# alibaba/EasyParallelLibrary

Hardware: AMD Instinct MI355X
Metric: samples_per_sec (higher is better)
Workload: dtype bf16; 1 GPU; model=bert-large, global_batch=128, seq_len=512, parallelism=dp1

## Files before the change

### csrc/kernels/attention.hip

```cpp

#include <hip/hip_runtime.h>
#include <cstdint>
#include <cstdlib>
#include <cstring>
#include <type_traits>

#include "attn_lds_image.h"

using bf16x8 = __attribute__((ext_vector_type(8))) short;
using bf16x4 = __attribute__((ext_vector_type(4))) short;
using f32x16 = __attribute__((ext_vector_type(16))) float;
using i32x2 = __attribute__((ext_vector_type(2))) int;
using u32x2 = __attribute__((ext_vector_type(2))) unsigned int;
using f32x2 = __attribute__((ext_vector_type(2))) float;
using f32x4 = __attribute__((ext_vector_type(4))) float;
using bf16v2 = __attribute__((ext_vector_type(2))) __bf16;

#define DEVI __device__ __forceinline__

namespace {

DEVI float bf2f(short u) {
  union { unsigned int i; float f; } v;
  v.i = ((unsigned int)(unsigned short)u) << 16;
  return v.f;
}

DEVI unsigned short f2bf(float f) {
  union { float f; unsigned int i; } v;
  v.f = f;
  unsigned int lsb = (v.i >> 16) & 1u;
  return (unsigned short)((v.i + 0x7fffu + lsb) >> 16);
}

DEVI unsigned int pack2(float a, float b) {
  return (unsigned int)f2bf(a) | ((unsigned int)f2bf(b) << 16);
}

DEVI int crow(int r, int hi) {
  return (r & 3) + 8 * (r >> 2) + 4 * hi;
}

DEVI unsigned int cvt_pk_bf16(float a, float b) {
  f32x2 f = {a, b};
  return __builtin_bit_cast(unsigned int,
                            __builtin_convertvector(f, bf16v2));
}

template <bool HW = false>
DEVI bf16x8 assemble_pfrag(const float* p) {
  unsigned int c0 = HW ? cvt_pk_bf16(p[0], p[1]) : pack2(p[0], p[1]);
  unsigned int c1 = HW ? cvt_pk_bf16(p[2], p[3]) : pack2(p[2], p[3]);
  unsigned int c2 = HW ? cvt_pk_bf16(p[4], p[5]) : pack2(p[4], p[5]);
  unsigned int c3 = HW ? cvt_pk_bf16(p[6], p[7]) : pack2(p[6], p[7]);
  i32x2 r = __builtin_amdgcn_permlane32_swap((int)c0, (int)c2, false, false);
  i32x2 s = __builtin_amdgcn_permlane32_swap((int)c1, (int)c3, false, false);
  union { unsigned int d[4]; bf16x8 v; } out;
  out.d[0] = (unsigned int)r[0];
  out.d[1] = (unsigned int)s[0];
  out.d[2] = (unsigned int)r[1];
  out.d[3] = (unsigned int)s[1];
  return out.v;
}

using attn_img::img_off;
using attn_img::img_pitch;
using attn_img::tr_frag;

template <bool TR, int D>
DEVI short* img_at(short (&img)[64][TR ? img_pitch<D>() : D + 8], int row,
                   int col) {
  return TR ? &img[0][0] + img_off<D>(row, col >> 3) : &img[row][col];
}

DEVI f32x16 load_rowconst(const float* c32, int hi) {
  f32x16 out;
#pragma unroll
  for (int g = 0; g < 4; ++g) {
    const f32x4 v = *reinterpret_cast<const f32x4*>(c32 + 8 * g + 4 * hi);
    out[4 * g + 0] = v[0];
    out[4 * g + 1] = v[1];
    out[4 * g + 2] = v[2];
    out[4 * g + 3] = v[3];
  }
  return out;
}

struct RowMask {
  int lo, hi_;
  DEVI RowMask(int64_t q0, int64_t seq, int64_t mykv, int causal) {
    const int64_t rows = seq - q0;
    hi_ = mykv >= seq ? 0 : (rows < 32 ? (int)rows : 32);
    const int64_t d = mykv - q0;
    lo = (causal && d > 0) ? (d < 32 ? (int)d : 32) : 0;
  }
  DEVI bool masked(int c) const { return c < lo || c >= hi_; }
};

DEVI void store_acc_bf16(short* p, const f32x16& acc, int hi) {
#pragma unroll
  for (int g = 0; g < 4; ++g) {
    u32x2 v = {cvt_pk_bf16(acc[4 * g], acc[4 * g + 1]),
               cvt_pk_bf16(acc[4 * g + 2], acc[4 * g + 3])};
    *reinterpret_cast<u32x2*>(p + 8 * g + 4 * hi) = v;
  }
}

DEVI int64_t sample_len(const int* seqlens, int64_t b, int64_t seq) {
  if (seqlens == nullptr) return seq;
  const int64_t n = __builtin_amdgcn_readfirstlane(seqlens[b]);
  return n < 0 ? 0 : (n > seq ? seq : n);
}

template <int D>
DEVI void zero_row(short* p, int hi) {
  const u32x2 z = {0u, 0u};
#pragma unroll
  for (int j = 0; j < D / 32; ++j)
#pragma unroll
    for (int g = 0; g < 4; ++g)
      *reinterpret_cast<u32x2*>(p + j * 32 + 8 * g + 4 * hi) = z;
}

DEVI void philox_round(unsigned int& c0, unsigned int& c1,
                       unsigned int& c2, unsigned int& c3,
                       unsigned int k0, unsigned int k1) {
  const unsigned int hi0 = __umulhi(0xD2511F53u, c0);
  const unsigned int lo0 = 0xD2511F53u * c0;
  const unsigned int hi1 = __umulhi(0xCD9E8D57u, c2);
  const unsigned int lo1 = 0xCD9E8D57u * c2;
  c0 = hi1 ^ c1 ^ k0;
  c1 = lo1;
  c2 = hi0 ^ c3 ^ k1;
  c3 = lo0;
}

DEVI void philox4x32(unsigned int c0, unsigned int c1, unsigned int c2,
                     unsigned int c3, unsigned int k0, unsigned int k1,
                     unsigned int out[4]) {
#pragma unroll
  for (int i = 0; i < 10; ++i) {
    philox_round(c0, c1, c2, c3, k0, k1);
    k0 += 0x9E3779B9u;
    k1 += 0xBB67AE85u;
  }
  out[0] = c0; out[1] = c1; out[2] = c2; out[3] = c3;
}


template <bool MASKED, bool DROP, int D>
DEVI void fwd_tile(const short (&ldsK)[64][D + 8],
                   const short (&ldsV)[D][72],
                   int sub, int64_t kvs, int64_t seq, int64_t myq,
                   float scale, int causal, const bf16x8 (&qfrag)[D / 16],
                   f32x16 (&ot)[D / 32], float& m, float& l, int lq,
                   int hi, unsigned int* maskrow, int64_t mask_w,
                   unsigned int seed0, unsigned int seed1,
                   unsigned int bh32, int drop_thresh, float inv_keep) {
  f32x16 st = {};
#pragma unroll
  for (int c = 0; c < D / 16; ++c) {
    bf16x8 kfrag =
        *reinterpret_cast<const bf16x8*>(&ldsK[sub + lq][hi * 8 + 16 * c]);
    st = __builtin_amdgcn_mfma_f32_32x32x16_bf16(kfrag, qfrag[c], st, 0, 0,
                                                 0);
  }
  float s[16];
  float tile_max = -1e30f;
#pragma unroll
  for (int r = 0; r < 16; ++r) {
    float sv = st[r] * scale;
    if (MASKED) {
      const int64_t kvg = kvs + crow(r, hi);
      if (kvg >= seq || (causal && kvg > myq)) sv = -1e30f;
    }
    s[r] = sv;
    tile_max = fmaxf(tile_max, sv);
  }
  tile_max = fmaxf(tile_max, __shfl_xor(tile_max, 32, 64));
  const float m_new = fmaxf(m, tile_max);
  const float alpha = __expf(m - m_new);
  float rowsum = 0.f;
#pragma unroll
  for (int r = 0; r < 16; ++r) {
    s[r] = __expf(s[r] - m_new);
    rowsum += s[r];
  }
  rowsum += __shfl_xor(rowsum, 32, 64);
  l = l * alpha + rowsum;
  m = m_new;
  if (DROP) {
    unsigned int rnd[4];
    philox4x32((unsigned int)myq,
               (unsigned int)(kvs >> 5) * 2u + (unsigned int)hi,
               bh32, 0x2E1B2137u, seed0, seed1, rnd);
    unsigned int mybits = 0;
#pragma unroll
    for (int r = 0; r < 16; ++r) {
      const unsigned int byte = (rnd[r >> 2] >> ((r & 3) * 8)) & 0xFFu;
      const bool keep = (int)byte >= drop_thresh;
      s[r] = keep ? s[r] * inv_keep : 0.f;
      mybits |= (unsigned int)keep << crow(r, hi);
    }
    const unsigned int word = mybits | __shfl_xor(mybits, 32, 64);
    if (hi == 0 && myq < seq)
      maskrow[myq * mask_w + (kvs >> 5)] = word;
  }
#pragma unroll
  for (int j = 0; j < D / 32; ++j)
#pragma unroll
    for (int r = 0; r < 16; ++r)
      ot[j][r] *= alpha;
  bf16x8 pf0 = assemble_pfrag<true>(&s[0]);
  bf16x8 pf1 = assemble_pfrag<true>(&s[8]);
#pragma unroll
  for (int kc = 0; kc < 2; ++kc) {
    bf16x8 pf = kc == 0 ? pf0 : pf1;
#pragma unroll
    for (int j = 0; j < D / 32; ++j) {
      bf16x8 vt = *reinterpret_cast<const bf16x8*>(
          &ldsV[j * 32 + lq][sub + kc * 16 + hi * 8]);
      ot[j] = __builtin_amdgcn_mfma_f32_32x32x16_bf16(vt, pf, ot[j], 0, 0,
                                                      0);
    }
  }
}

template <bool DROP, int D>
__global__ __launch_bounds__(256, D == 64 ? 3 : 2) void attn_fwd_kernel(
    const short* __restrict__ q, const short* __restrict__ k,
    const short* __restrict__ v, short* __restrict__ out,
    float* __restrict__ lse, int64_t seq, float scale, int causal,
    int64_t heads, int64_t in_sb, int64_t in_sh, int64_t in_ss,
    int64_t o_sb, int64_t o_sh, int64_t o_ss,
    unsigned int* __restrict__ mask, int64_t mask_w,
    unsigned long long seed, int drop_thresh, float inv_keep,
    const int* __restrict__ seqlens) {
  __shared__ short ldsV[2][D][72];
  __shared__ short ldsK[2][64][D + 8];
  const int lane = threadIdx.x & 63;
  const int wave = threadIdx.x >> 6;
  const int hi = lane >> 5;
  const int lq = lane & 31;
  const int64_t bh = causal ? (int64_t)blockIdx.x : (int64_t)blockIdx.y;
  const int64_t boff = (bh / heads) * in_sb + (bh % heads) * in_sh;
  const int64_t qb = causal ? (int64_t)gridDim.y - 1 - blockIdx.y
                            : (int64_t)blockIdx.x;
  const int64_t q0_blk = qb * 128;
  const int64_t q0 = q0_blk + wave * 32;
  const int64_t len = sample_len(seqlens, bh / heads, seq);
  const int64_t myq = q0 + lq;
  if (myq >= len && myq < seq) {
    zero_row<D>(out + (bh / heads) * o_sb + (bh % heads) * o_sh +
                    myq * o_ss, hi);
    if (hi == 0) lse[bh * seq + myq] = 0.f;
  }
  if (q0_blk >= len) return;
  const bool active = q0 < len;
  const short* qp = q + boff;
  const short* kp = k + boff;
  const short* vp = v + boff;

  const int64_t qrow = myq < len ? myq : len - 1;

  bf16x8 qfrag[D / 16];
#pragma unroll
  for (int c = 0; c < D / 16; ++c)
    qfrag[c] = *reinterpret_cast<const bf16x8*>(
        qp + qrow * in_ss + hi * 8 + 16 * c);

  f32x16 ot[D / 32] = {};
  float m = -1e30f, l = 0.f;

  const int64_t len64 = len & ~(int64_t)63;
  const int64_t bulk_end = causal ? (q0_blk < len64 ? q0_blk : len64) : len64;
  const int64_t blk_kv_end =
      causal ? (q0_blk + 128 < len ? q0_blk + 128 : len) : len;
  const int stage_kv = threadIdx.x & 63;
  const int stage_d0 = (threadIdx.x >> 6) * 8;

  bf16x8 pv[D / 32], pk[D / 32];
  auto load_tile = [&](int64_t kv0) {
    int64_t vrow = kv0 + stage_kv;
    if (vrow >= len) vrow = len - 1;
#pragma unroll
    for (int h2 = 0; h2 < D / 32; ++h2) {
      const int sd = stage_d0 + h2 * 32;
      pv[h2] = *reinterpret_cast<const bf16x8*>(vp + vrow * in_ss + sd);
      pk[h2] = *reinterpret_cast<const bf16x8*>(kp + vrow * in_ss + sd);
    }
  };
  auto write_tile = [&](int b) {
#pragma unroll
    for (int h2 = 0; h2 < D / 32; ++h2) {
      const int sd = stage_d0 + h2 * 32;
#pragma unroll
      for (int j = 0; j < 8; ++j)
        ldsV[b][sd + j][stage_kv] = pv[h2][j];
      *reinterpret_cast<bf16x8*>(&ldsK[b][stage_kv][sd]) = pk[h2];
    }
  };

  unsigned int* maskrow =
      DROP ? mask + bh * seq * mask_w : (unsigned int*)nullptr;
  const unsigned int seed0 = (unsigned int)seed;
  const unsigned int seed1 = (unsigned int)(seed >> 32);
  const unsigned int bh32 = (unsigned int)bh;

  int buf = 0;
  if (blk_kv_end > 0) load_tile(0);
  int64_t kv0 = 0;
  for (; kv0 < bulk_end; kv0 += 64) {
    write_tile(buf);
    __syncthreads();
    if (kv0 + 64 < blk_kv_end) load_tile(kv0 + 64);
#pragma unroll
    for (int sub = 0; sub < 64; sub += 32)
      fwd_tile<false, DROP, D>(ldsK[buf], ldsV[buf], sub, kv0 + sub, len,
                               myq, scale, causal, qfrag, ot, m, l, lq,
                               hi, maskrow, mask_w, seed0, seed1, bh32,
                               drop_thresh, inv_keep);
    buf ^= 1;
  }
  for (; kv0 < blk_kv_end; kv0 += 64) {
    write_tile(buf);
    __syncthreads();
    if (kv0 + 64 < blk_kv_end) load_tile(kv0 + 64);
    if (active) {
      const int64_t wave_kv_end = causal
          ? (q0 + 32 < len ? q0 + 32 : len) : len;
#pragma unroll
      for (int sub = 0; sub < 64; sub += 32) {
        const int64_t kvs = kv0 + sub;
        if (kvs >= wave_kv_end) break;
        fwd_tile<true, DROP, D>(ldsK[buf], ldsV[buf], sub, kvs, len, myq,
                                scale, causal, qfrag, ot, m, l, lq, hi,
                                maskrow, mask_w, seed0, seed1, bh32,
                                drop_thresh, inv_keep);
      }
    }
    buf ^= 1;
  }

  if (!active || myq >= len) return;
  const float inv_l = 1.f / l;
  short* op = out + (bh / heads) * o_sb + (bh % heads) * o_sh + myq * o_ss;
#pragma unroll
  for (int j = 0; j < D / 32; ++j)
    store_acc_bf16(op + j * 32, ot[j] * inv_l, hi);
  if (hi == 0) lse[bh * seq + myq] = m + __logf(l);
}

__global__ void attn_bwd_prep_kernel(const short* __restrict__ dout,
                                     const short* __restrict__ out,
                                     float* __restrict__ delta,
                                     int64_t rows, int64_t seq,
                                     int64_t heads, int64_t do_sb,
                                     int64_t do_sh, int64_t do_ss,
                                     int64_t o_sb, int64_t o_sh,
                                     int64_t o_ss) {
  const int lane = threadIdx.x & 63;
  const int waves_per_block = blockDim.x >> 6;
  for (int64_t row = (int64_t)blockIdx.x * waves_per_block +
                     (threadIdx.x >> 6);
       row < rows; row += (int64_t)gridDim.x * waves_per_block) {
    const int64_t bh = row / seq;
    const int64_t sq = row % seq;
    const short* dp = dout + (bh / heads) * do_sb + (bh % heads) * do_sh +
                      sq * do_ss;
    const short* op = out + (bh / heads) * o_sb + (bh % heads) * o_sh +
                      sq * o_ss;
    float acc = bf2f(dp[lane]) * bf2f(op[lane]);
#pragma unroll
    for (int off = 32; off > 0; off >>= 1)
      acc += __shfl_down(acc, off, 64);
    if (lane == 0) delta[row] = acc;
  }
}

__global__ __launch_bounds__(256) void attn_bwd_dkdv_kernel(
    const short* __restrict__ q, const short* __restrict__ k,
    const short* __restrict__ v, const short* __restrict__ dout,
    const float* __restrict__ lse, const float* __restrict__ delta,
    short* __restrict__ dk, short* __restrict__ dv, int64_t seq,
    float scale, int causal, int64_t heads, int64_t in_sb, int64_t in_sh,
    int64_t in_ss, int64_t do_sb, int64_t do_sh, int64_t do_ss,
    int64_t g_sb, int64_t g_sh, int64_t g_ss) {
  __shared__ short ldsQ[32][72];
  __shared__ short ldsDO[32][72];
  const int lane = threadIdx.x & 63;
  const int wave = threadIdx.x >> 6;
  const int hi = lane >> 5;
  const int lkv = lane & 31;
  const int64_t bh = blockIdx.y;
  const int64_t kv0_blk = (int64_t)blockIdx.x * 128;
  const int64_t kv0 = kv0_blk + wave * 32;
  const bool active = kv0 < seq;
  const int64_t boff = (bh / heads) * in_sb + (bh % heads) * in_sh;
  const short* qp = q + boff;
  const short* kp = k + boff;
  const short* vp = v + boff;
  const short* dop = dout + (bh / heads) * do_sb + (bh % heads) * do_sh;
  const float* lsep = lse + bh * seq;
  const float* dltp = delta + bh * seq;

  const int64_t mykv = kv0 + lkv;
  const int64_t kvrow = mykv < seq ? mykv : seq - 1;

  bf16x8 kfrag[4], vfrag[4];
#pragma unroll
  for (int c = 0; c < 4; ++c) {
    kfrag[c] = *reinterpret_cast<const bf16x8*>(
        kp + kvrow * in_ss + hi * 8 + 16 * c);
    vfrag[c] = *reinterpret_cast<const bf16x8*>(
        vp + kvrow * in_ss + hi * 8 + 16 * c);
  }

  f32x16 dvt0 = {}, dvt1 = {};
  f32x16 dkt0 = {}, dkt1 = {};

  const int stage_row = threadIdx.x >> 3;
  const int stage_seg = (threadIdx.x & 7) * 8;
  const int64_t q_start = causal ? (kv0_blk / 32) * 32 : 0;
  for (int64_t q0 = q_start; q0 < seq; q0 += 32) {
    __syncthreads();
    {
      int64_t qr = q0 + stage_row;
      if (qr >= seq) qr = seq - 1;
      *reinterpret_cast<bf16x8*>(&ldsQ[stage_row][stage_seg]) =
          *reinterpret_cast<const bf16x8*>(qp + qr * in_ss + stage_seg);
      *reinterpret_cast<bf16x8*>(&ldsDO[stage_row][stage_seg]) =
          *reinterpret_cast<const bf16x8*>(dop + qr * do_ss + stage_seg);
    }
    __syncthreads();
    if (!active || (causal && q0 + 31 < kv0)) continue;
    f32x16 st = {};
    f32x16 dpt = {};
#pragma unroll
    for (int c = 0; c < 4; ++c) {
      bf16x8 qf = *reinterpret_cast<const bf16x8*>(
          &ldsQ[lkv][hi * 8 + 16 * c]);
      bf16x8 dof = *reinterpret_cast<const bf16x8*>(
          &ldsDO[lkv][hi * 8 + 16 * c]);
      st = __builtin_amdgcn_mfma_f32_32x32x16_bf16(qf, kfrag[c], st, 0, 0,
                                                   0);
      dpt = __builtin_amdgcn_mfma_f32_32x32x16_bf16(dof, vfrag[c], dpt, 0,
                                                    0, 0);
    }
    float p[16], ds[16];
#pragma unroll
    for (int r = 0; r < 16; ++r) {
      const int64_t qg = q0 + crow(r, hi);
      const int64_t qgc = qg < seq ? qg : seq - 1;
      float sv = st[r] * scale;
      bool masked = qg >= seq || (causal && mykv > qg) || mykv >= seq;
      float pv = masked ? 0.f : __expf(sv - lsep[qgc]);
      p[r] = pv;
      ds[r] = masked ? 0.f : pv * (dpt[r] - dltp[qgc]) * scale;
    }
    bf16x8 pb0 = assemble_pfrag(&p[0]);
    bf16x8 pb1 = assemble_pfrag(&p[8]);
    bf16x8 db0 = assemble_pfrag(&ds[0]);
    bf16x8 db1 = assemble_pfrag(&ds[8]);
#pragma unroll
    for (int qc = 0; qc < 2; ++qc) {
      bf16x8 dot0, dot1, qt0, qt1;
#pragma unroll
      for (int j = 0; j < 8; ++j) {
        const int qr = qc * 16 + hi * 8 + j;
        dot0[j] = ldsDO[qr][lkv];
        dot1[j] = ldsDO[qr][32 + lkv];
        qt0[j] = ldsQ[qr][lkv];
        qt1[j] = ldsQ[qr][32 + lkv];
      }
      bf16x8 pb = qc == 0 ? pb0 : pb1;
      bf16x8 db = qc == 0 ? db0 : db1;
      dvt0 = __builtin_amdgcn_mfma_f32_32x32x16_bf16(dot0, pb, dvt0, 0, 0,
                                                     0);
      dvt1 = __builtin_amdgcn_mfma_f32_32x32x16_bf16(dot1, pb, dvt1, 0, 0,
                                                     0);
      dkt0 = __builtin_amdgcn_mfma_f32_32x32x16_bf16(qt0, db, dkt0, 0, 0,
                                                     0);
      dkt1 = __builtin_amdgcn_mfma_f32_32x32x16_bf16(qt1, db, dkt1, 0, 0,
                                                     0);
    }
  }

  if (!active || mykv >= seq) return;
  const int64_t goff = (bh / heads) * g_sb + (bh % heads) * g_sh +
                       mykv * g_ss;
  short* dkp = dk + goff;
  short* dvp = dv + goff;
#pragma unroll
  for (int r = 0; r < 16; ++r) {
    dvp[crow(r, hi)] = (short)f2bf(dvt0[r]);
    dvp[32 + crow(r, hi)] = (short)f2bf(dvt1[r]);
    dkp[crow(r, hi)] = (short)f2bf(dkt0[r]);
    dkp[32 + crow(r, hi)] = (short)f2bf(dkt1[r]);
  }
}


template <bool MASKED, bool DROP, int D>
DEVI void dv_tile(const short (&ldsQ)[64][D + 8],
                  const short (&ldsDO)[64][D + 8],
                  int sub, int64_t q0, int64_t seq, int64_t mykv,
                  float scale, int causal, const float* lsep,
                  const bf16x8 (&kfrag)[D / 16], f32x16 (&dvt)[D / 32],
                  int lkv, int hi, const unsigned int* maskrow,
                  int64_t mask_w, float inv_keep) {
  f32x16 st = {};
#pragma unroll
  for (int c = 0; c < D / 16; ++c) {
    bf16x8 qf = *reinterpret_cast<const bf16x8*>(
        &ldsQ[sub + lkv][hi * 8 + 16 * c]);
    st = __builtin_amdgcn_mfma_f32_32x32x16_bf16(qf, kfrag[c], st, 0, 0, 0);
  }
  float p[16];
#pragma unroll
  for (int r = 0; r < 16; ++r) {
    const int64_t qg = q0 + crow(r, hi);
    const int64_t qgc = qg < seq ? qg : seq - 1;
    if (MASKED) {
      bool masked = qg >= seq || (causal && mykv > qg) || mykv >= seq;
      p[r] = masked ? 0.f : __expf(st[r] * scale - lsep[qgc]);
    } else {
      p[r] = __expf(st[r] * scale - lsep[qg]);
    }
    if (DROP) {
      const int64_t kvc = mykv < seq ? mykv : seq - 1;
      const unsigned int w = maskrow[qgc * mask_w + (kvc >> 5)];
      p[r] *= ((w >> (kvc & 31)) & 1u) ? inv_keep : 0.f;
    }
  }
  bf16x8 pb0 = assemble_pfrag(&p[0]);
  bf16x8 pb1 = assemble_pfrag(&p[8]);
#pragma unroll
  for (int qc = 0; qc < 2; ++qc) {
    bf16x8 pb = qc == 0 ? pb0 : pb1;
#pragma unroll
    for (int dj = 0; dj < D / 32; ++dj) {
      bf16x8 dot;
#pragma unroll
      for (int j = 0; j < 8; ++j) {
        const int qr = sub + qc * 16 + hi * 8 + j;
        dot[j] = ldsDO[qr][dj * 32 + lkv];
      }
      dvt[dj] =
          __builtin_amdgcn_mfma_f32_32x32x16_bf16(dot, pb, dvt[dj], 0, 0, 0);
    }
  }
}

template <bool MASKED, bool DROP, int D>
DEVI void dk_tile(const short (&ldsQ)[64][D + 8],
                  const short (&ldsDO)[64][D + 8],
                  int sub, int64_t q0, int64_t seq, int64_t mykv,
                  float scale, int causal, const float* lsep,
                  const float* dltp, const bf16x8 (&kfrag)[D / 16],
                  const bf16x8 (&vfrag)[D / 16], f32x16 (&dkt)[D / 32],
                  int lkv, int hi, const unsigned int* maskrow,
                  int64_t mask_w, float inv_keep) {
  f32x16 st = {};
  f32x16 dpt = {};
#pragma unroll
  for (int c = 0; c < D / 16; ++c) {
    bf16x8 qf = *reinterpret_cast<const bf16x8*>(
        &ldsQ[sub + lkv][hi * 8 + 16 * c]);
    bf16x8 dof = *reinterpret_cast<const bf16x8*>(
        &ldsDO[sub + lkv][hi * 8 + 16 * c]);
    st = __builtin_amdgcn_mfma_f32_32x32x16_bf16(qf, kfrag[c], st, 0, 0, 0);
    dpt = __builtin_amdgcn_mfma_f32_32x32x16_bf16(dof, vfrag[c], dpt, 0, 0,
                                                  0);
  }
  float ds[16];
#pragma unroll
  for (int r = 0; r < 16; ++r) {
    const int64_t qg = q0 + crow(r, hi);
    const int64_t qgc = qg < seq ? qg : seq - 1;
    float dp = dpt[r];
    if (DROP) {
      const int64_t kvc = mykv < seq ? mykv : seq - 1;
      const unsigned int w = maskrow[qgc * mask_w + (kvc >> 5)];
      dp *= ((w >> (kvc & 31)) & 1u) ? inv_keep : 0.f;
    }
    if (MASKED) {
      bool masked = qg >= seq || (causal && mykv > qg) || mykv >= seq;
      float pv = masked ? 0.f : __expf(st[r] * scale - lsep[qgc]);
      ds[r] = masked ? 0.f : pv * (dp - dltp[qgc]) * scale;
    } else {
      float pv = __expf(st[r] * scale - lsep[qg]);
      ds[r] = pv * (dp - dltp[qg]) * scale;
    }
  }
  bf16x8 db0 = assemble_pfrag(&ds[0]);
  bf16x8 db1 = assemble_pfrag(&ds[8]);
#pragma unroll
  for (int qc = 0; qc < 2; ++qc) {
    bf16x8 db = qc == 0 ? db0 : db1;
#pragma unroll
    for (int dj = 0; dj < D / 32; ++dj) {
      bf16x8 qt;
#pragma unroll
      for (int j = 0; j < 8; ++j) {
        const int qr = sub + qc * 16 + hi * 8 + j;
        qt[j] = ldsQ[qr][dj * 32 + lkv];
      }
      dkt[dj] =
          __builtin_amdgcn_mfma_f32_32x32x16_bf16(qt, db, dkt[dj], 0, 0, 0);
    }
  }
}

template <bool MASKED, bool DROP, int D>
DEVI void dv_tile_tr(const short* imgQ, const short* imgDO,
                     const float* lseL, int sub, int64_t q0, int64_t seq,
                     int64_t mykv, float scale, int causal,
                     const bf16x8 (&kfrag)[D / 16], f32x16 (&dvt)[D / 32],
                     int lkv, int hi, const unsigned int* maskrow,
                     int64_t mask_w, float inv_keep) {
  f32x16 st = load_rowconst(lseL, hi);
#pragma unroll
  for (int c = 0; c < D / 16; ++c) {
    bf16x8 qf = *reinterpret_cast<const bf16x8*>(
        imgQ + img_off<D>(sub + lkv, 2 * c + hi));
    st = __builtin_amdgcn_mfma_f32_32x32x16_bf16(qf, kfrag[c], st, 0, 0, 0);
  }
  const float c2 = scale * 1.44269504088896341f;
  const RowMask rm(q0, seq, mykv, causal);
  float p[16];
#pragma unroll
  for (int r = 0; r < 16; ++r) {
    if (MASKED)
      p[r] = rm.masked(crow(r, hi)) ? 0.f
                                    : __builtin_amdgcn_exp2f(st[r] * c2);
    else
      p[r] = __builtin_amdgcn_exp2f(st[r] * c2);
    if (DROP) {
      const int64_t qg = q0 + crow(r, hi);
      const int64_t qgc = qg < seq ? qg : seq - 1;
      const int64_t kvc = mykv < seq ? mykv : seq - 1;
      const unsigned int w = maskrow[qgc * mask_w + (kvc >> 5)];
      p[r] *= ((w >> (kvc & 31)) & 1u) ? inv_keep : 0.f;
    }
  }
  bf16x8 pb0 = assemble_pfrag<true>(&p[0]);
  bf16x8 pb1 = assemble_pfrag<true>(&p[8]);
  const int lane = hi * 32 + lkv;
#pragma unroll
  for (int qc = 0; qc < 2; ++qc) {
    bf16x8 pb = qc == 0 ? pb0 : pb1;
#pragma unroll
    for (int dj = 0; dj < D / 32; ++dj) {
// ... 975 lines not shown
```

Baseline: 725.4 samples/s.

## Restructure attention forward with lazy rescale, exp2 softmax, transposed V image, staged output

The forward attention tile folds the softmax scale into an exp2 constant and applies it in an FMA. The running max and accumulator are now rescaled only when a wave sees the max grow past a threshold, and the cross-half row reductions are deferred to the end via permlane32 swaps. V staging moves to a row-segmented load into a precomputed LDS image read through a transposed fragment helper, replacing per-element scattered LDS writes. The output is staged through LDS so the global stores are coalesced. This adds extra syncthreads and relies on the lazy-rescale threshold staying numerically safe in fp32.

```diff
diff --git a/csrc/kernels/attention.hip b/csrc/kernels/attention.hip
--- a/csrc/kernels/attention.hip
+++ b/csrc/kernels/attention.hip
@@ -148,11 +148,19 @@
 }
 
 
+DEVI void both_halves(unsigned int x, unsigned int& lo, unsigned int& hi_) {
+  const i32x2 r = __builtin_amdgcn_permlane32_swap((int)x, (int)x, false,
+                                                   false);
+  lo = (unsigned int)r[0];
+  hi_ = (unsigned int)r[1];
+}
+
+constexpr float kRescaleThr = 8.f;
+
 template <bool MASKED, bool DROP, int D>
-DEVI void fwd_tile(const short (&ldsK)[64][D + 8],
-                   const short (&ldsV)[D][72],
+DEVI void fwd_tile(const short (&ldsK)[64][D + 8], const short* imgV,
                    int sub, int64_t kvs, int64_t seq, int64_t myq,
-                   float scale, int causal, const bf16x8 (&qfrag)[D / 16],
+                   float c2, int causal, const bf16x8 (&qfrag)[D / 16],
                    f32x16 (&ot)[D / 32], float& m, float& l, int lq,
                    int hi, unsigned int* maskrow, int64_t mask_w,
                    unsigned int seed0, unsigned int seed1,
@@ -169,7 +177,7 @@
   float tile_max = -1e30f;
 #pragma unroll
   for (int r = 0; r < 16; ++r) {
-    float sv = st[r] * scale;
+    float sv = st[r];
     if (MASKED) {
       const int64_t kvg = kvs + crow(r, hi);
       if (kvg >= seq || (causal && kvg > myq)) sv = -1e30f;
@@ -177,18 +185,31 @@
     s[r] = sv;
     tile_max = fmaxf(tile_max, sv);
   }
-  tile_max = fmaxf(tile_max, __shfl_xor(tile_max, 32, 64));
-  const float m_new = fmaxf(m, tile_max);
-  const float alpha = __expf(m - m_new);
+  {
+    unsigned int a, b;
+    both_halves(__builtin_bit_cast(unsigned int, tile_max), a, b);
+    tile_max = fmaxf(__builtin_bit_cast(float, a),
+                     __builtin_bit_cast(float, b));
+  }
+  if (__builtin_amdgcn_ballot_w64((tile_max - m) * c2 > kRescaleThr) != 0) {
+    const float m_new = fmaxf(m, tile_max);
+    const float alpha = __builtin_amdgcn_exp2f((m - m_new) * c2);
+    m = m_new;
+    l *= alpha;
+#pragma unroll
+    for (int j = 0; j < D / 32; ++j)
+#pragma unroll
+      for (int r = 0; r < 16; ++r)
+        ot[j][r] *= alpha;
+  }
+  const float nmc = -m * c2;
   float rowsum = 0.f;
 #pragma unroll
   for (int r = 0; r < 16; ++r) {
-    s[r] = __expf(s[r] - m_new);
+    s[r] = __builtin_amdgcn_exp2f(__builtin_fmaf(s[r], c2, nmc));
     rowsum += s[r];
   }
-  rowsum += __shfl_xor(rowsum, 32, 64);
-  l = l * alpha + rowsum;
-  m = m_new;
+  l += rowsum;
   if (DROP) {
     unsigned int rnd[4];
     philox4x32((unsigned int)myq,
@@ -202,15 +223,11 @@
       s[r] = keep ? s[r] * inv_keep : 0.f;
       mybits |= (unsigned int)keep << crow(r, hi);
     }
-    const unsigned int word = mybits | __shfl_xor(mybits, 32, 64);
+    unsigned int wlo, whi;
+    both_halves(mybits, wlo, whi);
     if (hi == 0 && myq < seq)
-      maskrow[myq * mask_w + (kvs >> 5)] = word;
-  }
-#pragma unroll
-  for (int j = 0; j < D / 32; ++j)
-#pragma unroll
-    for (int r = 0; r < 16; ++r)
-      ot[j][r] *= alpha;
+      maskrow[myq * mask_w + (kvs >> 5)] = wlo | whi;
+  }
   bf16x8 pf0 = assemble_pfrag<true>(&s[0]);
   bf16x8 pf1 = assemble_pfrag<true>(&s[8]);
 #pragma unroll
@@ -218,8 +235,7 @@
     bf16x8 pf = kc == 0 ? pf0 : pf1;
 #pragma unroll
     for (int j = 0; j < D / 32; ++j) {
-      bf16x8 vt = *reinterpret_cast<const bf16x8*>(
-          &ldsV[j * 32 + lq][sub + kc * 16 + hi * 8]);
+      bf16x8 vt = tr_frag<D>(imgV, sub + 16 * kc, j, hi * 32 + lq);
       ot[j] = __builtin_amdgcn_mfma_f32_32x32x16_bf16(vt, pf, ot[j], 0, 0,
                                                       0);
     }
@@ -236,8 +252,9 @@
     unsigned int* __restrict__ mask, int64_t mask_w,
     unsigned long long seed, int drop_thresh, float inv_keep,
     const int* __restrict__ seqlens) {
-  __shared__ short ldsV[2][D][72];
-  __shared__ short ldsK[2][64][D + 8];
+  __shared__ __attribute__((aligned(16))) short
+      ldsV[2][64 * img_pitch<D>()];
+  __shared__ __attribute__((aligned(16))) short ldsK[2][64][D + 8];
   const int lane = threadIdx.x & 63;
   const int wave = threadIdx.x >> 6;
   const int hi = lane >> 5;
@@ -271,34 +288,42 @@
 
   f32x16 ot[D / 32] = {};
   float m = -1e30f, l = 0.f;
+  const float c2 = scale * 1.44269504088896341f;
 
   const int64_t len64 = len & ~(int64_t)63;
   const int64_t bulk_end = causal ? (q0_blk < len64 ? q0_blk : len64) : len64;
   const int64_t blk_kv_end =
       causal ? (q0_blk + 128 < len ? q0_blk + 128 : len) : len;
-  const int stage_kv = threadIdx.x & 63;
-  const int stage_d0 = (threadIdx.x >> 6) * 8;
-
-  bf16x8 pv[D / 32], pk[D / 32];
+
+  const int stage_row = threadIdx.x >> 3;
+  const int stage_seg = (threadIdx.x & 7) * 8;
+  bf16x8 pv[2][D / 64], pk[2][D / 64];
   auto load_tile = [&](int64_t kv0) {
-    int64_t vrow = kv0 + stage_kv;
-    if (vrow >= len) vrow = len - 1;
-#pragma unroll
-    for (int h2 = 0; h2 < D / 32; ++h2) {
-      const int sd = stage_d0 + h2 * 32;
-      pv[h2] = *reinterpret_cast<const bf16x8*>(vp + vrow * in_ss + sd);
-      pk[h2] = *reinterpret_cast<const bf16x8*>(kp + vrow * in_ss + sd);
+#pragma unroll
+    for (int half = 0; half < 2; ++half) {
+      int64_t vrow = kv0 + stage_row + half * 32;
+      if (vrow >= len) vrow = len - 1;
+#pragma unroll
+      for (int s = 0; s < D / 64; ++s) {
+        const int col = stage_seg + s * 64;
+        pv[half][s] =
+            *reinterpret_cast<const bf16x8*>(vp + vrow * in_ss + col);
+        pk[half][s] =
+            *reinterpret_cast<const bf16x8*>(kp + vrow * in_ss + col);
+      }
     }
   };
   auto write_tile = [&](int b) {
 #pragma unroll
-    for (int h2 = 0; h2 < D / 32; ++h2) {
-      const int sd = stage_d0 + h2 * 32;
-#pragma unroll
-      for (int j = 0; j < 8; ++j)
-        ldsV[b][sd + j][stage_kv] = pv[h2][j];
-      *reinterpret_cast<bf16x8*>(&ldsK[b][stage_kv][sd]) = pk[h2];
-    }
+    for (int half = 0; half < 2; ++half)
+#pragma unroll
+      for (int s = 0; s < D / 64; ++s) {
+        const int row = stage_row + half * 32;
+        const int col = stage_seg + s * 64;
+        *reinterpret_cast<bf16x8*>(
+            &ldsV[b][img_off<D>(row, col >> 3)]) = pv[half][s];
+        *reinterpret_cast<bf16x8*>(&ldsK[b][row][col]) = pk[half][s];
+      }
   };
 
   unsigned int* maskrow =
@@ -317,8 +342,8 @@
 #pragma unroll
     for (int sub = 0; sub < 64; sub += 32)
       fwd_tile<false, DROP, D>(ldsK[buf], ldsV[buf], sub, kv0 + sub, len,
-                               myq, scale, causal, qfrag, ot, m, l, lq,
-                               hi, maskrow, mask_w, seed0, seed1, bh32,
+                               myq, c2, causal, qfrag, ot, m, l, lq, hi,
+                               maskrow, mask_w, seed0, seed1, bh32,
                                drop_thresh, inv_keep);
     buf ^= 1;
   }
@@ -334,7 +359,7 @@
         const int64_t kvs = kv0 + sub;
         if (kvs >= wave_kv_end) break;
         fwd_tile<true, DROP, D>(ldsK[buf], ldsV[buf], sub, kvs, len, myq,
-                                scale, causal, qfrag, ot, m, l, lq, hi,
+                                c2, causal, qfrag, ot, m, l, lq, hi,
                                 maskrow, mask_w, seed0, seed1, bh32,
                                 drop_thresh, inv_keep);
       }
@@ -342,13 +367,30 @@
     buf ^= 1;
   }
 
-  if (!active || myq >= len) return;
+  {
+    unsigned int a, b;
+    both_halves(__builtin_bit_cast(unsigned int, l), a, b);
+    l = __builtin_bit_cast(float, a) + __builtin_bit_cast(float, b);
+  }
   const float inv_l = 1.f / l;
-  short* op = out + (bh / heads) * o_sb + (bh % heads) * o_sh + myq * o_ss;
+  short* ob = out + (bh / heads) * o_sb + (bh % heads) * o_sh;
+  short* ldsO = &ldsK[0][0][0] + wave * 32 * (D + 8);
+  __syncthreads();
 #pragma unroll
   for (int j = 0; j < D / 32; ++j)
-    store_acc_bf16(op + j * 32, ot[j] * inv_l, hi);
-  if (hi == 0) lse[bh * seq + myq] = m + __logf(l);
+    store_acc_bf16(ldsO + lq * (D + 8) + j * 32, ot[j] * inv_l, hi);
+  __syncthreads();
+  constexpr int LPR = D / 8;
+#pragma unroll
+  for (int r0 = 0; r0 < 32; r0 += 64 / LPR) {
+    const int r = r0 + lane / LPR;
+    const int col = (lane % LPR) * 8;
+    const bf16x8 piece =
+        *reinterpret_cast<const bf16x8*>(ldsO + r * (D + 8) + col);
+    if (q0 + r < len)
+      *reinterpret_cast<bf16x8*>(ob + (q0 + r) * o_ss + col) = piece;
+  }
+  if (hi == 0 && myq < len) lse[bh * seq + myq] = m * scale + __logf(l);
 }
 
 __global__ void attn_bwd_prep_kernel(const short* __restrict__ dout,
```

Result: faster. 733.8 samples/s, median of 6 (+1.2%).
